# neverorfrog/vehicle-control

Hardware: AMD Instinct MI355X
Metric: MPC solves/sec (batched, N=20) (higher is better)
Workload: dtype f64; 1 GPU; C2 kinematic-bicycle LTV-MPC, B=1024 per GPU, N=20, fp64; batch_per_gpu=1024, global_batch=1024, horizon=20, parallelism=dp1 (independent shards)

## Files before the change

### vehicle-control_amd/csrc/kin_ltv.hip

```cpp
#include <hip/hip_runtime.h>

#include <cstdint>

#include "vc_kernels.hpp"
#include "vc_models.hpp"
#include "vcmpc.h"

#ifndef KIN_NU_TOL
#define KIN_NU_TOL 1e-10
#endif
#ifndef KIN_EARLY_F
#define KIN_EARLY_F 100.0
#endif
#ifndef KIN_EARLY_ROUNDS
#define KIN_EARLY_ROUNDS 2
#endif
#ifndef KIN_TAPIA_F
#define KIN_TAPIA_F 1.02
#endif
#ifndef KIN_DUAL_TOL
#define KIN_DUAL_TOL 1e-12
#endif
#ifndef KIN_AL_RHO
#define KIN_AL_RHO 1e1
#endif
#ifndef KIN_DOT_CH
#define KIN_DOT_CH 8
#endif
#ifndef KIN_UPDATE
#define KIN_UPDATE 1
#endif
#ifndef KIN_RSQ_HALLEY
#define KIN_RSQ_HALLEY 1
#endif
#ifndef KIN_STAT_CHECK
#define KIN_STAT_CHECK 0
#endif
#ifndef KIN_STEP_F
#define KIN_STEP_F 0.99
#endif
#ifndef KIN_SOLVE_CH
#define KIN_SOLVE_CH 8
#endif
#ifndef KIN_PANEL_CH
#define KIN_PANEL_CH 6
#endif

namespace vc {
namespace {

__device__ __forceinline__ double lane_bcast(double v, int src) {
  const int lo = __builtin_amdgcn_readlane(__double2loint(v), src);
  const int hi = __builtin_amdgcn_readlane(__double2hiint(v), src);
  return __hiloint2double(hi, lo);
}
__device__ int amdgcn_writelane(int v, int lane, int old) __asm("llvm.amdgcn.writelane.i32");
__device__ __forceinline__ double lane_put(double old, double v, int dst) {
  const int lo = amdgcn_writelane(__double2loint(v), dst, __double2loint(old));
  const int hi = amdgcn_writelane(__double2hiint(v), dst, __double2hiint(old));
  return __hiloint2double(hi, lo);
}
template <int K>
__device__ __forceinline__ double dpp_row_shr(double v, double ident) {
  const int lo = __builtin_amdgcn_update_dpp(__double2loint(ident), __double2loint(v), 0x110 + K, 0xf, 0xf, false);
  const int hi = __builtin_amdgcn_update_dpp(__double2hiint(ident), __double2hiint(v), 0x110 + K, 0xf, 0xf, false);
  return __hiloint2double(hi, lo);
}
template <typename Op>
__device__ __forceinline__ double wave_reduce(double v, double ident, Op op) {
  v = op(v, dpp_row_shr<1>(v, ident));
  v = op(v, dpp_row_shr<2>(v, ident));
  v = op(v, dpp_row_shr<4>(v, ident));
  v = op(v, dpp_row_shr<8>(v, ident));
  return op(op(lane_bcast(v, 15), lane_bcast(v, 31)), op(lane_bcast(v, 47), lane_bcast(v, 63)));
}
__device__ __forceinline__ double wave_sum(double v) {
  return wave_reduce(v, 0.0, [](double a, double b) { return a + b; });
}
__device__ __forceinline__ double wave_max(double v) {
  return wave_reduce(v, -__builtin_inf(), [](double a, double b) { return fmax(a, b); });
}
__device__ __forceinline__ double wave_min(double v) {
  return wave_reduce(v, __builtin_inf(), [](double a, double b) { return fmin(a, b); });
}
__device__ __forceinline__ void wave_sync() {
  asm volatile("" ::: "memory");
  __builtin_amdgcn_wave_barrier();
  asm volatile("" ::: "memory");
}
__device__ __forceinline__ void fence() { __builtin_amdgcn_sched_barrier(0); }
__device__ __forceinline__ int lane_opaque(int lane) {
  asm volatile("" : "+v"(lane));
  return lane;
}
__device__ __forceinline__ uint32_t lane_range_pick(uint32_t in, int other, int lo, int hi) {
  uint32_t r;
  asm("s_bfm_b64 vcc, %3, %4\n\t"
      "v_mov_b32_e32 %0, %2\n\tv_cndmask_b32_e32 %0, %0, %1, vcc"
      : "=&v"(r)
      : "v"(in), "i"(other), "i"(hi - lo), "i"(lo)
      : "vcc");
  return r;
}
__device__ __forceinline__ void no_hoist() { asm volatile("" ::: "memory"); }

using lds_cdouble = const __attribute__((address_space(3))) double;
__device__ __forceinline__ lds_cdouble* lds_opaque(const double* p) {
  uint32_t a = (uint32_t)(uintptr_t)(lds_cdouble*)p;
  asm volatile("" : "+v"(a));
  return (lds_cdouble*)(uintptr_t)a;
}

#ifdef VC_TIMING
#define VC_TSTAMP(var) \
  fence();              \
  const uint64_t var = __builtin_amdgcn_s_memtime(); \
  fence();
#define VC_TACC(slot, t0) \
  {                      \
    fence();             \
    tacc[slot] += __builtin_amdgcn_s_memtime() - (t0); \
    fence();             \
  }
#else
#define VC_TSTAMP(var)
#define VC_TACC(slot, t0)
#endif
enum { T_SWEEP = 0, T_SETUP, T_RESID, T_BUILD, T_CHOL, T_SOLVE, T_UPDATE, T_POLISH, T_OUT, T_S2, T_S3, T_S4, T_PAL, T_PPASS, T_NUPD, T_UCYC, T_NDROP, T_CFAIL, T_CRM, T_CADD, T_R0CHG, T_STEP, T_TOTAL, T_NSLOT };


template <int N>
struct Dims {
  static constexpr int n = 2 * N;
  static constexpr int NC = 2 * (N - 1);
  static constexpr int LD = n + 1;
  static_assert(n <= 64 && N >= 2, "one wavefront per problem needs 2 <= N <= 32");
};

template <int n>
__host__ __device__ constexpr int lc_base(int k) {
  static_assert(n % 2 == 0, "even n");
  return k * (n - 1) - k * (k - 1) / 2 + (k + 1) / 2;
}
template <int n>
__host__ __device__ constexpr int lc_start(int k) {
  return lc_base<n>(k) + k;
}

template <int N>
struct Smem {
  using D = Dims<N>;
  static constexpr int LC_DUMMY = lc_start<D::n>(D::n);
  static constexpr int LC_ZERO = LC_DUMMY + 1;
  double G[D::NC + 3][D::LD];
  double H[D::n + 1][D::LD];
  alignas(16) double Lc[LC_ZERO + 1];
  alignas(16) double zrow[48];
  double xb[N + 1][KIN_NX + 1];
  double jac[N + 1][9];
  double ub[D::n];
  double kap[N], ds[N];
  union {
    struct {
      double vz[64];
      double vc[64];
    };
    alignas(16) double tb2[128];
  };
  double dinv[64];
};

template <int N>
__host__ __device__ constexpr int crow_stage(int r) {
  return r < N - 1 ? r + 1 : r - (N - 1) + 1;
}

template <int LEN, int SA, int SB, int CH = KIN_DOT_CH>
__device__ __forceinline__ double lds_dot(lds_cdouble* a, lds_cdouble* b) {
  constexpr int NCH = (LEN + CH - 1) / CH;
  double ca[2][CH], cb[2][CH];
  auto fetch = [&](int c, int buf) {
#pragma unroll
    for (int q = 0; q < CH; ++q) {
      const int i = c * CH + q;
      ca[buf][q] = (i < LEN) ? a[i * SA] : 0.0;
      cb[buf][q] = (i < LEN) ? b[i * SB] : 0.0;
    }
  };
  double a0 = 0.0, a1 = 0.0;
  fetch(0, 0);
#pragma unroll
  for (int c = 0; c < NCH; ++c) {
    if (c + 1 < NCH) fetch(c + 1, (c + 1) & 1);
    fence();
#pragma unroll
    for (int q = 0; q < CH; q += 2) {
      a0 += ca[c & 1][q] * cb[c & 1][q];
      a1 += ca[c & 1][q + 1] * cb[c & 1][q + 1];
    }
  }
  fence();
  return a0 + a1;
}

template <int N>
__device__ double grow_dot(const Smem<N>& s, int lane) {
  constexpr int NC = Dims<N>::NC;
  const int r = lane < NC ? lane : 0;
  const double a = lds_dot<2 * (N - 1), 1, 1>(lds_opaque(&s.G[r][0]), lds_opaque(&s.vz[0]));
  return lane < NC ? a : 0.0;
}

template <int N>
__device__ double gt_dot(const Smem<N>& s, int lane) {
  constexpr int n = Dims<N>::n, NC = Dims<N>::NC, LD = Dims<N>::LD;
  const int j = lane < n ? lane : 0;
  const double a = lds_dot<NC, LD, 1>(lds_opaque(&s.G[0][j]), lds_opaque(&s.vc[0]));
  return lane < n ? a : 0.0;
}


template <int N>
__device__ double h_dot(const Smem<N>& s, int lane) {
  constexpr int n = Dims<N>::n;
  const int j = lane < n ? lane : 0;
  return lds_dot<n, 1, 1>(lds_opaque(&s.H[j][0]), lds_opaque(&s.vz[0]));
}

__device__ __forceinline__ void kin_sincos(double x, double& sn, double& cs) {
  const double n = __builtin_rint(x * 6.36619772367581382433e-01);
  const double y = fma(-n, 6.07710050650619224932e-11, fma(-n, 1.57079632673412561417e+00, x));
  const double z = y * y;
  const double rs = fma(z, fma(z, fma(z, fma(z, 1.58969099521155010221e-10, -2.50507602534068634195e-08),
                                      2.75573137070700676789e-06), -1.98412698298579493134e-04),
                        8.33333333332248946124e-03);
  const double sk = fma(z * y, fma(z, rs, -1.66666666666666324348e-01), y);
  const double rc = z * fma(z, fma(z, fma(z, fma(z, fma(z, -1.13596475577881948265e-11, 2.08757232129817482790e-09),
                                                  -2.75573143513906633035e-07), 2.48015872894767294178e-05),
                                   -1.38888888888741095749e-03), 4.16666666666666019037e-02);
  const double hz = 0.5 * z, w = 1.0 - hz;
  const double ck = w + (((1.0 - w) - hz) + z * rc);
  const int q = int(n) & 3;
  const double a = (q & 1) ? ck : sk, b = (q & 1) ? sk : ck;
  sn = (q & 2) ? -a : a;
  cs = ((q + 1) & 2) ? -b : b;
}

__device__ __forceinline__ double rsq_nr(double d) {
  double inv = __builtin_amdgcn_rsq(d);
#if KIN_RSQ_HALLEY
  const double e = fma(-d, inv * inv, 1.0);
  return fma(inv * e, fma(0.375, e, 0.5), inv);
#else
  inv = inv * (1.5 - 0.5 * d * inv * inv);
  inv = inv * (1.5 - 0.5 * d * inv * inv);
  return inv;
#endif
}

template <int N>
__device__ __forceinline__ void store_rows(const double (&Mr)[Dims<N>::n], Smem<N>& s, int lane) {
}

template <int N>
__device__ double chol_solve(const double (&Lr)[Dims<N>::n], const Smem<N>& s, double b, int lane) {
  constexpr int n = Dims<N>::n;
  constexpr int CH = KIN_SOLVE_CH;
  static_assert(n % CH == 0, "backward prefetch chunks");
  const int row = lane < n ? lane : 0;
  lds_cdouble* col = lds_opaque(&s.Lc[lc_base<n>(row)]);
  const double dj = s.dinv[row];
  double acc = b;
#pragma unroll
  for (int k = 0; k < n; ++k) acc -= Lr[k] * lane_bcast(acc * dj, k);
  acc *= dj;
  double x = 0.0;
  double lk[2][CH];
  lds_cdouble* zero = lds_opaque(&s.zrow[0]);
  auto fetch = [&](int c, int buf) {
    lds_cdouble* src = row < n - 1 - c * CH ? col : zero;
#pragma unroll
    for (int q = 0; q < CH; ++q) lk[buf][q] = src[n - 1 - c * CH - q];
  };
  fetch(0, 0);
#pragma unroll
  for (int c = 0; c < n / CH; ++c) {
    if (c + 1 < n / CH) fetch(c + 1, (c + 1) & 1);
    fence();
#pragma unroll
    for (int q = 0; q < CH; ++q) {
      const int k = n - 1 - c * CH - q;
      const double xk = lane_bcast(acc * dj, k);
      x = lane_put(x, xk, k);
      acc -= lk[c & 1][q] * xk;
    }
    fence();
  }
  return x;
}

enum { ROWS_G = 0, ROWS_E = 1 };
template <int N, int KIND>
__host__ __device__ constexpr int row_extent(int r) {
  if (KIND == ROWS_G) return r < Dims<N>::NC ? 2 * crow_stage<N>(r) : 0;
  return r < N ? 2 * (r + 1) : (r < N + 2 ? 2 * N : 0);
}
template <int N, int KIND>
__host__ __device__ constexpr int gram_rows() {
  return KIND == ROWS_G ? Dims<N>::NC : N + 2;
}
template <int N, int KIND>
__host__ __device__ constexpr bool kstep_hits(int ks, int I) {
  for (int q = 0; q < 4; ++q)
    if (row_extent<N, KIND>(4 * ks + q) > 16 * I) return true;
  return false;
}

using d4 = __attribute__((ext_vector_type(4))) double;
using d2 = __attribute__((ext_vector_type(2))) double;
template <int N>
struct Tiles {
  static constexpr int n = Dims<N>::n, NB = (n + 15) / 16, NT = NB * (NB + 1) / 2, BLD = 16 * NB + 2;
  static constexpr int count(bool full) { return full ? NB * NB : NT; }
};

template <int N, int KIND, bool FULL>
__device__ __forceinline__ void gram_mfma(d4 (&acc)[Tiles<N>::count(FULL)], const double* rows, const double* w,
                                          int lane) {
  constexpr int n = Dims<N>::n, LD = Dims<N>::LD, NB = Tiles<N>::NB;
  constexpr int KS = (gram_rows<N, KIND>() + 3) / 4;
  lane = lane_opaque(lane);
  const int lr = lane >> 4, lc = lane & 15;
  lds_cdouble* R = lds_opaque(rows);
  lds_cdouble* W = lds_opaque(w);
  double gk[KS][NB], wk[KS];
#pragma unroll
  for (int ks = 0; ks < KS; ++ks) {
    const int r = 4 * ks + lr;
    wk[ks] = W[r];
#pragma unroll
    for (int J = 0; J < NB; ++J) {
      const int c = 16 * J + lc;
      gk[ks][J] = R[r * LD + (c < n ? c : n)];
    }
  }
  fence();
#pragma unroll
  for (int ks = 0; ks < KS; ++ks) {
#pragma unroll
    for (int I = 0, t = 0; I < NB; ++I) {
      const double a = wk[ks] * gk[ks][I];
#pragma unroll
      for (int J = 0; J < (FULL ? NB : I + 1); ++J, ++t)
        if (kstep_hits<N, KIND>(ks, I > J ? I : J))
          acc[t] = __builtin_amdgcn_mfma_f64_16x16x4f64(a, gk[ks][J], acc[t], 0, 0, 0);
    }
  }
}

template <int N, bool FULL>
__device__ __forceinline__ void tiles_to_rows(double (&Mr)[Dims<N>::n], const d4 (&acc)[Tiles<N>::count(FULL)],
                                              Smem<N>& s, int lane) {
  constexpr int n = Dims<N>::n, NB = Tiles<N>::NB, BLD = Tiles<N>::BLD;
  static_assert(16 * BLD <= Smem<N>::LC_DUMMY, "transpose buffer must fit the factor storage");
  static_assert(16 * NB <= 48, "zero row length");
  lane = lane_opaque(lane);
  const int lr = lane >> 4, lc = lane & 15;
  double* buf = &s.Lc[0];
  const int myI = lane >> 4;
#pragma unroll
  for (int I = 0, t0 = 0; I < NB; ++I, t0 += FULL ? NB : I) {
    wave_sync();
#pragma unroll
    for (int J = 0; J < (FULL ? NB : I + 1); ++J) {
#pragma unroll
      for (int q = 0; q < 4; ++q) buf[(lr + 4 * q) * BLD + 16 * J + lc] = acc[t0 + J][q];
    }
    wave_sync();
    using lds_cd2 = const __attribute__((address_space(3))) d2;
    lds_cd2* brow = (lds_cd2*)lds_opaque(myI == I ? &buf[lc * BLD] : &s.zrow[0]);
#pragma unroll
    for (int i = 0; i < n; i += 2) {
      const int iend = FULL ? n : 16 * (I + 1);
      if (i < iend) {
        const d2 p = brow[i / 2];
        if (I == 0) { Mr[i] = p.x; Mr[i + 1] = p.y; }
        else { Mr[i] += p.x; Mr[i + 1] += p.y; }
      } else if (I == 0) {
        Mr[i] = 0.0;
        Mr[i + 1] = 0.0;
      }
    }
  }
  wave_sync();
}

template <int N>
__device__ __forceinline__ void build_normal_acc(d4 (&acc)[Tiles<N>::NT], Smem<N>& s, double wb, double hjj, int lane) {
  constexpr int n = Dims<N>::n, LD = Dims<N>::LD, NB = Tiles<N>::NB;
  static_assert(4 * ((Dims<N>::NC + 3) / 4) <= Dims<N>::NC + 2, "G zero rows cover the last k-step");
  lane = lane_opaque(lane);
  const int lr = lane >> 4, lc = lane & 15;
  const int jd = lane < n ? lane : n;
  s.H[jd][jd] = hjj + wb;
  wave_sync();
  {
    lds_cdouble* H = lds_opaque(&s.H[0][0]);
#pragma unroll
    for (int I = 0, t = 0; I < NB; ++I) {
#pragma unroll
      for (int J = 0; J <= I; ++J, ++t) {
        const int c = 16 * J + lc < n ? 16 * J + lc : n;
#pragma unroll
        for (int q = 0; q < 4; ++q) {
          const int r0 = 16 * I + 4 * q;
          acc[t][q] = r0 < n ? H[(r0 + lr) * LD + c] : 0.0;
        }
      }
    }
  }
  s.H[jd][jd] = hjj;
  gram_mfma<N, ROWS_G, false>(acc, &s.G[0][0], &s.vc[0], lane);
}

template <int N>
__device__ __forceinline__ void build_normal_mfma(double (&Mr)[Dims<N>::n], Smem<N>& s, double wb, double hjj,
                                                  int lane) {
  d4 acc[Tiles<N>::NT];
  build_normal_acc<N>(acc, s, wb, hjj, lane);
  tiles_to_rows<N, false>(Mr, acc, s, lane);
}

template <int N>
__device__ bool factor_blocked(double (&Mr)[Dims<N>::n], d4 (&acc)[Tiles<N>::NT], Smem<N>& s, int lane) {
  constexpr int n = Dims<N>::n, NB = Tiles<N>::NB;
  constexpr int DUMMY = Smem<N>::LC_DUMMY;
  static_assert(NB == 3 && n > 32 && n <= 40, "three panels, the last one at most 8 wide");
  static_assert(lc_start<n>(16) + 16 * 18 <= DUMMY, "panel 0/1 transpose buffer inside the factor storage");
  static_assert((lc_start<n>(16) & 1) == 0, "16-byte aligned transpose buffer");
  lane = lane_opaque(lane);
  const int lr = lane >> 4, lc = lane & 15, myI = lane >> 4;
  bool ok = true;
  double pa, pb, pc, pi1, pl21, pi2;
  using lds_double = __attribute__((address_space(3))) double;
  using lds_char = __attribute__((address_space(3))) char;
  const uint32_t lane8 = 8u * uint32_t(lane);
  auto col_store = [&](int k, double v) {
    const uint32_t off = lane_range_pick(lane8, 8 * (DUMMY - lc_base<n>(k)), k, n);
    *(lds_double*)((lds_char*)&s.Lc[lc_base<n>(k)] + off) = v;
  };
  auto part = [&](int p, int k) {
    if (p == 0) {
      pa = lane_bcast(Mr[k], k);
      pb = lane_bcast(Mr[k], k + 1);
      pc = lane_bcast(Mr[k + 1], k + 1);
      pi1 = rsq_nr(pa);
    } else if (p == 1) {
      pl21 = pb * pi1;
      const double d2 = fma(-pl21, pl21, pc);
      pi2 = rsq_nr(d2);
      ok = ok && (pa > 0.0) && (d2 > 0.0);
    } else {
      const double x = Mr[k] * pi1;
      const double y = fma(-x, pl21, Mr[k + 1]) * pi2;
      Mr[k] = x;
      Mr[k + 1] = y;
      col_store(k, x);
      col_store(k + 1, y);
      s.dinv[k] = pi1;
      s.dinv[k + 1] = pi2;
    }
  };
  using lds_cd2 = const __attribute__((address_space(3))) d2;
#pragma unroll
  for (int p = 0; p < NB; ++p) {
    const int c0 = 16 * p, c1 = (16 * p + 16 < n) ? 16 * p + 16 : n, W = c1 - c0;
    double* tb = p < 2 ? &s.Lc[lc_start<n>(16)] : &s.tb2[0];
    const int TS = p < 2 ? 18 : 10;
#pragma unroll
    for (int i = c0; i < c1; ++i) Mr[i] = 0.0;
#pragma unroll
    for (int I = p; I < NB; ++I) {
      const int t = I * (I + 1) / 2 + p;
      wave_sync();
#pragma unroll
      for (int q = 0; q < 4; ++q) {
        const int r = lr + 4 * q;
        if (4 * q < W)
          tb[(lc < W ? r * TS + lc : 8 * TS + lc)] = acc[t][q];
      }
      wave_sync();
      lds_cd2* src = (lds_cd2*)lds_opaque(myI == I && lc < W ? &tb[lc * TS] : &s.zrow[0]);
#pragma unroll
      for (int i = 0; i < W; i += 2) {
        const d2 v = src[i / 2];
        Mr[c0 + i] += v.x;
        Mr[c0 + i + 1] += v.y;
      }
    }
    wave_sync();
    part(0, c0);
    part(1, c0);
    part(2, c0);
#pragma unroll
    for (int k = c0; k + 2 < c1; k += 2) {
      wave_sync();
      fence();
      const double x = Mr[k], y = Mr[k + 1];
      const double* cA = &s.Lc[lc_base<n>(k)];
      const double* cB = &s.Lc[lc_base<n>(k + 1)];
      constexpr int CH = KIN_PANEL_CH;
      const int J0 = k + 4, NCH = (c1 - J0 + CH - 1) / CH;
      double u0[2][CH], u1[2][CH];
      auto load = [&](int ch, int buf) {
#pragma unroll
        for (int q = 0; q < CH; ++q) {
          const int j = J0 + ch * CH + q;
          u0[buf][q] = j < c1 ? cA[j] : 0.0;
          u1[buf][q] = j < c1 ? cB[j] : 0.0;
        }
      };
      if (NCH > 0) load(0, 0);
#pragma unroll
      for (int j = k + 2; j < k + 4; ++j)
        Mr[j] = fma(-y, lane_bcast(y, j), fma(-x, lane_bcast(x, j), Mr[j]));
      part(0, k + 2);
#pragma unroll
      for (int ch = 0; ch < NCH; ++ch) {
        if (ch + 1 < NCH) load(ch + 1, (ch + 1) & 1);
        fence();
#pragma unroll
        for (int q = 0; q < CH; ++q) {
          const int j = J0 + ch * CH + q;
          if (j < c1) Mr[j] = fma(-y, u1[ch & 1][q], fma(-x, u0[ch & 1][q], Mr[j]));
        }
        if (ch + 1 < 3) part(ch + 1, k + 2);
        fence();
      }
#pragma unroll
      for (int pp = NCH + 1; pp < 3; ++pp) {
        part(pp, k + 2);
        fence();
      }
    }
    wave_sync();
    if (p + 1 < NB) {
      lds_cdouble* Lc = lds_opaque(&s.Lc[0]);
      lds_cdouble* Z = lds_opaque(&s.zrow[0]);
#pragma unroll
      for (int ks = 0; ks < W / 4; ++ks) {
        const int kk = c0 + 4 * ks + lr;
        double op[NB];
#pragma unroll
        for (int I = p + 1; I < NB; ++I) {
          const int jj = 16 * I + lc;
          op[I] = jj < n ? Lc[lc_base<n>(kk) + jj] : Z[0];
        }
#pragma unroll
        for (int I = p + 1; I < NB; ++I) {
#pragma unroll
          for (int J = p + 1; J <= I; ++J) {
            const int t = I * (I + 1) / 2 + J;
            acc[t] = __builtin_amdgcn_mfma_f64_16x16x4f64(-op[I], op[J], acc[t], 0, 0, 0);
          }
        }
      }
    }
  }
#pragma unroll
  for (int k = 0; k < n; ++k) Mr[k] = lane_opaque(lane) > k ? Mr[k] : 0.0;
  store_rows<N>(Mr, s, lane);
  wave_sync();
  return ok;
}

__device__ __forceinline__ double wave_prefix(double v, int lane) {
  v += dpp_row_shr<1>(v, 0.0);
  v += dpp_row_shr<2>(v, 0.0);
  v += dpp_row_shr<4>(v, 0.0);
  v += dpp_row_shr<8>(v, 0.0);
  const double r0 = lane_bcast(v, 15), r1 = lane_bcast(v, 31), r2 = lane_bcast(v, 47);
  return v + (lane >= 16 ? r0 : 0.0) + (lane >= 32 ? r1 : 0.0) + (lane >= 48 ? r2 : 0.0);
}

template <int N>
__device__ bool factor_update(double (&Mr)[Dims<N>::n], Smem<N>& s, int upd, int j, bool fixed, double sqrho,
                              int lane) {
  constexpr int n = Dims<N>::n;
  constexpr int DUMMY = Smem<N>::LC_DUMMY, ZERO = Smem<N>::LC_ZERO;
  lane = lane_opaque(lane);
  const int row = lane < n ? lane : 0;
  auto below = [&](int k, int other) { return lane > k && lane < n ? lc_base<n>(k) + lane : other; };
  double z;
  if (upd == 1) {
    z = s.Lc[below(j, ZERO)];
    wave_sync();
    s.Lc[below(j, DUMMY)] = 0.0;
    s.Lc[lane < j ? lc_base<n>(lane) + j : DUMMY] = 0.0;
    s.Lc[lc_start<n>(j)] = 1.0;
    s.dinv[j] = 1.0;
  } else {
    z = (lane < n && !fixed) ? sqrho * s.G[j][lane < n ? lane : n] : 0.0;
  }
  wave_sync();
  {
    lds_cdouble* L = lds_opaque(&s.Lc[0]);
#pragma unroll
    for (int k = 0; k < n; ++k) Mr[k] = L[below(k, ZERO)];
  }
  const double dj = s.dinv[row];
  double acc = z;
#pragma unroll
  for (int k = 0; k < n; ++k) acc -= Mr[k] * lane_bcast(acc * dj, k);
  const double y = lane < n ? acc * dj : 0.0;
  const double t = 1.0 + wave_prefix(y * y, lane);
  const double sk = sqrt(t / (t - y * y)), ck = y / t;
  const bool ok = __ballot(!(sk > 0.5 && sk < 1e150)) == 0ull;
  wave_sync();
  if (lane < n) {
    s.Lc[lc_start<n>(row)] *= sk;
    s.dinv[row] = dj / sk;
  }
  s.tb2[2 * lane] = ck;
  s.tb2[2 * lane + 1] = sk;
  wave_sync();
  {
    using lds_cd2 = const __attribute__((address_space(3))) d2;
    lds_cd2* cs = (lds_cd2*)lds_opaque(&s.tb2[0]);
    double w = z;
#pragma unroll
    for (int k = 0; k < n - 1; ++k) {
      const double yk = lane_bcast(y, k);
      const d2 c = cs[k];
      w = lane_put(w, 0.0, k);
      const double l = Mr[k];
      w = fma(-yk, l, w);
      Mr[k] = fma(c.x, w, l) * c.y;
    }
  }
#pragma unroll
  for (int k = 0; k < n - 1; ++k) s.Lc[below(k, DUMMY)] = Mr[k];
  wave_sync();
  return ok;
}

struct Side {
  double lo, hi, slo, shi, llo, lhi;
  bool hasLo, hasHi;
};

}

template <int N>
__global__ __launch_bounds__(64) void kin_ltv_kernel(KinLtvArgs A) {
  using D = Dims<N>;
  constexpr int n = D::n, NC = D::NC;
  __shared__ Smem<N> s;
  const int lane = threadIdx.x;
  const int b = xcd_problem(blockIdx.x, A.B);
  if (b >= A.B) return;
  const vc_kin_mpc& W = A.w;
#ifdef VC_TIMING
  uint64_t tacc[T_NSLOT] = {};
#endif
  VC_TSTAMP(t_all0)

  if (lane < n) s.ub[lane] = A.ubar[(size_t)b * n + lane];
  if (lane < N) {
    s.kap[lane] = A.kappa[(size_t)b * N + lane];
    s.ds[lane] = A.ds[(size_t)b * N + lane];
  }
  if (lane < KIN_NX) s.xb[0][lane] = A.x0[(size_t)b * KIN_NX + lane];
  for (int i = lane; i < 2 * D::LD; i += 64) (&s.G[NC][0])[i] = 0.0;
  if (lane < 48) s.zrow[lane] = 0.0;
  if (lane == 0) s.Lc[Smem<N>::LC_ZERO] = 0.0;
  wave_sync();

  VC_TSTAMP(t_sweep0)
  constexpr int LD = Dims<N>::LD;
  double* E = &s.H[0][0];
  bool finite = true;
  {
    double x[KIN_NX];
#pragma unroll
    for (int i = 0; i < KIN_NX; ++i) x[i] = s.xb[0][i];
#pragma unroll 1
    for (int k = 0; k < N; ++k) {
      const double u2[2] = {s.ub[2 * k], s.ub[2 * k + 1]};
      const double h = s.ds[k];
      double f[KIN_NX];
      {
        double sn, cs;
        kin_sincos((lane & 1) ? x[1] : x[4], sn, cs);
        const double se = lane_bcast(sn, 0), ce = lane_bcast(cs, 0);
        const double sd = lane_bcast(sn, 1), cd = lane_bcast(cs, 1);
        const double kap = s.kap[k];
        const double rho = 1.0 - x[3] * kap;
        const int r4 = lane & 3;
        const double num = r4 == 0 ? se : (r4 == 1 ? sd : rho);
        const double den = r4 == 0 ? ce : (r4 == 1 ? cd * A.L : (r4 == 2 ? ce : x[0] * ce));
        const double quo = num * rcp_nr(den);
        const double te = lane_bcast(quo, 0), tdl = lane_bcast(quo, 1);
        const double rc = lane_bcast(quo, 2), q = lane_bcast(quo, 3);
        f[0] = q * u2[0];
        f[1] = q * u2[1];
        f[2] = 1.0;
        f[3] = rho * te;
        f[4] = tdl * rc - kap;
        f[5] = q;
      }
#pragma unroll
      for (int i = 0; i < KIN_NX; ++i) x[i] += h * f[i];
      if (lane == 0) {
#pragma unroll
        for (int i = 0; i < KIN_NX; ++i) s.xb[k + 1][i] = x[i];
      }
    }
#pragma unroll
    for (int i = 0; i < KIN_NX; ++i) finite = finite && isfinite(x[i]);
  }
  wave_sync();
  if (lane < N) {
    const double ey = s.xb[lane + 1][3];
    double cw, lin;
    if (lane + 1 < N) {
      const double hs = s.ds[lane + 1];
      const double td = W.w_dev * hs;
      double tb = W.w_b * hs;
      asm volatile("" : "+v"(tb));
      cw = td;
      lin = ey * td;
      if (ey < W.ey_min) { cw = __builtin_fma(W.w_dev, hs, tb); lin = __builtin_fma(ey - W.ey_min, tb, lin); }
      if (ey > W.ey_max) { cw = cw + tb; lin = __builtin_fma(ey - W.ey_max, tb, lin); }
    } else {
      cw = W.w_ey;
      lin = W.w_ey * ey;
    }
    s.vc[lane] = 2.0 * cw;
    s.vz[lane] = 2.0 * lin;
  }
  wave_sync();
  VC_TACC(T_SWEEP, t_sweep0)
  VC_TSTAMP(t_s20)
  {
    const int k = lane < N ? lane : 0;
    double xk[KIN_NX];
#pragma unroll
    for (int i = 0; i < KIN_NX; ++i) xk[i] = s.xb[k][i];
    const KinJac J = kin_spatial_jac(xk, s.kap[k], A.L);
    double* jr = s.jac[lane < N ? lane : N];
    jr[0] = J.q; jr[1] = J.qv; jr[2] = J.qey; jr[3] = J.qep;
    jr[4] = J.J33; jr[5] = J.J34; jr[6] = J.J41; jr[7] = J.J43; jr[8] = J.J44;
    if (A.obs.n > 0 && lane >= 1 && lane < N) {
      double p, q;
      obstacle_ey_model<double>(A.obs, xk[2], xk[3], W.w_obs * s.ds[k], p, q);
      s.vc[k - 1] += q;
      s.vz[k - 1] += p;
    }
  }
  wave_sync();
  VC_TACC(T_S2, t_s20)
  VC_TSTAMP(t_s30)
  double gj = 0.0;
  double cv = 0, cd = 0, cey = 0, cep = 0, ct = 0;
  {
    const int jcol = lane < n ? lane : n;
    double jn[9], hn, an, wn;
    auto fetch = [&](int k) {
#pragma unroll
      for (int q = 0; q < 9; ++q) jn[q] = s.jac[k][q];
      hn = s.ds[k]; an = s.ub[2 * k]; wn = s.ub[2 * k + 1];
    };
    fetch(0);
#pragma unroll 1
    for (int k = 0; k < N; ++k) {
      double J[9];
#pragma unroll
      for (int q = 0; q < 9; ++q) J[q] = jn[q];
      const double h = hn, a = an, w = wn;
      const double lin2 = s.vz[k];
      if (k + 1 < N) fetch(k + 1);
      const double dq = J[1] * cv + J[2] * cey + J[3] * cep;
      const double ncv = cv + h * a * dq + (lane == 2 * k ? h * J[0] : 0.0);
      const double ncd = cd + h * w * dq + (lane == 2 * k + 1 ? h * J[0] : 0.0);
      const double ncey = cey + h * (J[4] * cey + J[5] * cep);
      const double ncep = cep + h * (J[6] * cd + J[7] * cey + J[8] * cep);
      ct += h * dq;
      cv = ncv; cd = ncd; cey = ncey; cep = ncep;
      const bool has = k + 1 <= N - 1;
      s.G[has ? k : NC + 2][jcol] = cv;
      s.G[has ? (N - 1) + k : NC + 2][jcol] = cd;
      E[k * LD + jcol] = cey;
      gj += lin2 * cey;
    }
    E[N * LD + jcol] = cv;
    E[(N + 1) * LD + jcol] = cep;
  }
  wave_sync();
  VC_TACC(T_S3, t_s30)
  VC_TSTAMP(t_s40)
  double Hr[n];
  double hjj;
  {
    const double vN = s.xb[N][0];
    const double cwv = (vN >= W.v_max) ? W.w_v : 0.0;
    gj += 2.0 * cwv * (vN - W.v_max) * cv;
    gj += 2.0 * W.w_epsi * s.xb[N][4] * cep;
    gj += W.w_time * ct;
    if (lane < 4) s.vc[N + lane] = lane == 0 ? 2.0 * cwv : (lane == 1 ? 2.0 * W.w_epsi : 0.0);
    for (int i = lane; i < 2 * LD; i += 64) E[(N + 2) * LD + i] = 0.0;
    wave_sync();
    d4 acc[Tiles<N>::count(true)];
#pragma unroll
    for (int t = 0; t < Tiles<N>::count(true); ++t) acc[t] = d4{0.0, 0.0, 0.0, 0.0};
    gram_mfma<N, ROWS_E, true>(acc, E, &s.vc[0], lane);
    tiles_to_rows<N, true>(Hr, acc, s, lane);
  }
  const int kq = lane >> 1;
  double dself = 2.0 * A.qp.prox, dm2 = 0.0, dp2 = 0.0;
  if (lane < n) {
    if (lane & 1) {
      dself += 2.0 * W.w_w;
      gj += 2.0 * W.w_w * s.ub[lane];
    } else {
      if (kq >= 1) {
        dself += 2.0 * W.w_a; dm2 = -2.0 * W.w_a;
        gj += 2.0 * W.w_a * (s.ub[lane] - s.ub[lane - 2]);
      }
      if (kq <= N - 2) {
        dself += 2.0 * W.w_a; dp2 = -2.0 * W.w_a;
        gj -= 2.0 * W.w_a * (s.ub[lane + 2] - s.ub[lane]);
      }
    }
  }
  gj = (lane < n) ? gj : 0.0;
  {
    const int j = lane < n ? lane : n;
#pragma unroll
    for (int i = 0; i < n; ++i) s.H[j][i] = Hr[i];
    s.H[j][n] = 0.0;
    s.H[j][j] += dself;
    s.H[j][j >= 2 ? j - 2 : j] += dm2;
    s.H[j][j + 2 < n ? j + 2 : j] += dp2;
    hjj = lane < n ? s.H[j][j] : 0.0;
  }
  wave_sync();
  if (A.mode == 1) {
    if (lane < n) {
#pragma unroll
      for (int i = 0; i < n; ++i) A.H_out[((size_t)b * n + lane) * n + i] = s.H[lane][i];
      A.g_out[(size_t)b * n + lane] = gj;
    }
    return;
  }

  VC_TACC(T_S4, t_s40)
  VC_TSTAMP(t_setup0)
  Side bx, cs;
  {
    const bool isw = lane & 1;
    const double u = (lane < n) ? s.ub[lane] : 0.0;
    bx.lo = (isw ? W.w_min : W.a_min) - u;
    bx.hi = (isw ? W.w_max : W.a_max) - u;
    const double tr = isw ? A.qp.trust_w : A.qp.trust_a;
    if (tr > 0.0) {
      bx.lo = fmax(bx.lo, -tr);
      bx.hi = fmin(bx.hi, tr);
    }
    bx.hasLo = bx.hasHi = (lane < n);
    const int st = crow_stage<N>(lane < NC ? lane : 0);
    if (lane < N - 1) {
      cs.lo = W.v_min - s.xb[st][0];
      cs.hi = 0.0;
      cs.hasLo = true; cs.hasHi = false;
    } else if (lane < NC) {
      cs.lo = W.delta_min - s.xb[st][1];
      cs.hi = W.delta_max - s.xb[st][1];
      cs.hasLo = cs.hasHi = true;
    } else {
      cs.lo = cs.hi = 0.0;
      cs.hasLo = cs.hasHi = false;
    }
  }
  const double mtot = double(4 * N + 3 * (N - 1));
  double scale, hdiag_max;
  {
    double m = fabs(gj);
    if (bx.hasLo) m = fmax(m, fabs(bx.lo));
    if (bx.hasHi) m = fmax(m, fabs(bx.hi));
    if (cs.hasLo) m = fmax(m, fabs(cs.lo));
    if (cs.hasHi) m = fmax(m, fabs(cs.hi));
    scale = 1.0 + wave_max(m);
    hdiag_max = fmax(wave_max(hjj), 1.0);
  }
  double z = 0.0;
  bx.slo = bx.hasLo ? fmax(-bx.lo, 1.0) : 1.0;
  bx.shi = bx.hasHi ? fmax(bx.hi, 1.0) : 1.0;
  bx.llo = bx.hasLo ? 1.0 : 0.0;
  bx.lhi = bx.hasHi ? 1.0 : 0.0;
  cs.slo = cs.hasLo ? fmax(-cs.lo, 1.0) : 1.0;
  cs.shi = cs.hasHi ? fmax(cs.hi, 1.0) : 1.0;
  cs.llo = cs.hasLo ? 1.0 : 0.0;
  cs.lhi = cs.hasHi ? 1.0 : 0.0;

  VC_TACC(T_SETUP, t_setup0)
  const int max_iter = A.qp.max_iter;
  const double tol = A.qp.tol * scale;
  int it = 0;
  bool converged = false, chol_fail = false, near = false;
  double last_res = 0.0, last_mu = 0.0;
  double Mr[n];
  double rd = 0.0, rlo_b = 0.0, rhi_b = 0.0, rlo_c = 0.0, rhi_c = 0.0;
  auto true_residuals = [&]() {
    wave_sync();
    s.vz[lane] = (lane < n) ? z : 0.0;
    s.vc[lane] = (lane < NC) ? (cs.lhi - cs.llo) : 0.0;
    wave_sync();
    const double yc = grow_dot<N>(s, lane);
    rd = (lane < n) ? (h_dot<N>(s, lane) + gj + (bx.lhi - bx.llo) + gt_dot<N>(s, lane)) : 0.0;
    rlo_b = bx.hasLo ? (z - bx.lo - bx.slo) : 0.0;
    rhi_b = bx.hasHi ? (bx.hi - z - bx.shi) : 0.0;
    rlo_c = cs.hasLo ? (yc - cs.lo - cs.slo) : 0.0;
    rhi_c = cs.hasHi ? (cs.hi - yc - cs.shi) : 0.0;
  };
  auto max_residual = [&]() {
    return wave_max(fmax(fmax(fabs(rd), fmax(fabs(rlo_b), fabs(rhi_b))), fmax(fabs(rlo_c), fabs(rhi_c))));
  };
  int tapb = 0;
  const double tol_early = KIN_EARLY_F > 0.0 ? fmax(tol, KIN_EARLY_F * tol) : tol;
  int e_set = 0;
#ifdef VC_TIMING
  uint64_t e_fmask = 0;
  bool e_row = false, e_have = false;
#endif
  double tol_cur = tol_early;
  bool polished = false, pchol_fail = false;
  int rounds = 0;
#pragma unroll 1
  for (;;) {
  if (finite) {
#pragma unroll 1
    for (;;) {
      no_hoist();
      VC_TSTAMP(t_res0)
      if (it == 0) true_residuals();
      const double mu = wave_sum(bx.slo * bx.llo + bx.shi * bx.lhi + cs.slo * cs.llo + cs.shi * cs.lhi) / mtot;
      double res = max_residual();
      if (it > 0 && res <= tol_cur && mu <= tol_cur) {
        true_residuals();
        res = max_residual();
      }
      converged = res <= tol_cur && mu <= tol_cur;
      last_res = res;
      last_mu = mu;
      if (converged || it >= max_iter || !isfinite(res) || !isfinite(mu)) break;
      ++it;
      const double wlo_b = bx.hasLo ? bx.llo / bx.slo : 0.0;
      const double whi_b = bx.hasHi ? bx.lhi / bx.shi : 0.0;
      const double wlo_c = cs.hasLo ? cs.llo / cs.slo : 0.0;
      const double whi_c = cs.hasHi ? cs.lhi / cs.shi : 0.0;
      wave_sync();
      s.vc[lane] = (lane < NC) ? wlo_c + whi_c : 0.0;
      wave_sync();
      VC_TACC(T_RESID, t_res0)
      VC_TSTAMP(t_build0)
      d4 nacc[Tiles<N>::NT];
      build_normal_acc<N>(nacc, s, wlo_b + whi_b, hjj, lane);
      VC_TACC(T_BUILD, t_build0)
      VC_TSTAMP(t_chol0)
      const bool chol_ok = factor_blocked<N>(Mr, nacc, s, lane);
      VC_TACC(T_CHOL, t_chol0)
      if (!chol_ok) {
        chol_fail = true;
        near = res <= 1e-6 * scale && mu <= tol;
        break;
      }
#ifdef VC_TIMING
      const uint64_t t_sol_before = tacc[T_SOLVE];
#endif
      VC_TSTAMP(t_step0)
      const double islo_b = bx.hasLo ? rcp_nr(bx.slo) : 0.0, ishi_b = bx.hasHi ? rcp_nr(bx.shi) : 0.0;
      const double islo_c = cs.hasLo ? rcp_nr(cs.slo) : 0.0, ishi_c = cs.hasHi ? rcp_nr(cs.shi) : 0.0;
      const double illo_b = bx.hasLo ? rcp_nr(bx.llo) : 0.0, ilhi_b = bx.hasHi ? rcp_nr(bx.lhi) : 0.0;
      const double illo_c = cs.hasLo ? rcp_nr(cs.llo) : 0.0, ilhi_c = cs.hasHi ? rcp_nr(cs.lhi) : 0.0;
      double sm = 0.0, pp1 = 0.0, pp2 = 0.0, pp3 = 0.0, pp4 = 0.0;
#pragma unroll 1
      for (int pass = 0; pass < 2; ++pass) {
        no_hoist();
        const double rclo_b = bx.slo * bx.llo + pp1 - sm, rchi_b = bx.shi * bx.lhi + pp2 - sm;
        const double rclo_c = cs.slo * cs.llo + pp3 - sm, rchi_c = cs.shi * cs.lhi + pp4 - sm;
        const double eb = (bx.hasHi ? (-rchi_b * ishi_b - whi_b * rhi_b) : 0.0) +
                          (bx.hasLo ? (rclo_b * islo_b + wlo_b * rlo_b) : 0.0);
        const double ec = (cs.hasHi ? (-rchi_c * ishi_c - whi_c * rhi_c) : 0.0) +
                          (cs.hasLo ? (rclo_c * islo_c + wlo_c * rlo_c) : 0.0);
        wave_sync();
        s.vc[lane] = (lane < NC) ? ec : 0.0;
        wave_sync();
        const double rhs = (lane < n) ? (-rd - eb - gt_dot<N>(s, lane)) : 0.0;
        VC_TSTAMP(t_sol0)
        const double dz = chol_solve<N>(Mr, s, rhs, lane);
        VC_TACC(T_SOLVE, t_sol0)
        wave_sync();
        s.vz[lane] = (lane < n) ? dz : 0.0;
        wave_sync();
        const double dyc = grow_dot<N>(s, lane);
        const double d1 = bx.hasLo ? dz + rlo_b : 0.0;
        const double d2 = bx.hasLo ? (-rclo_b * islo_b - wlo_b * (dz + rlo_b)) : 0.0;
        const double d3 = bx.hasHi ? rhi_b - dz : 0.0;
        const double d4 = bx.hasHi ? (-rchi_b * ishi_b - whi_b * (rhi_b - dz)) : 0.0;
        const double e1 = cs.hasLo ? dyc + rlo_c : 0.0;
        const double e2 = cs.hasLo ? (-rclo_c * islo_c - wlo_c * (dyc + rlo_c)) : 0.0;
        const double e3 = cs.hasHi ? rhi_c - dyc : 0.0;
        const double e4 = cs.hasHi ? (-rchi_c * ishi_c - whi_c * (rhi_c - dyc)) : 0.0;
        const double tmax = wave_max(fmax(fmax(fmax(-d1 * islo_b, -d2 * illo_b), fmax(-d3 * ishi_b, -d4 * ilhi_b)),
                                          fmax(fmax(-e1 * islo_c, -e2 * illo_c), fmax(-e3 * ishi_c, -e4 * ilhi_c))));
        const double amax = 1.0 / fmax(1.0, tmax);
        if (pass == 0) {
          const double mua = wave_sum((bx.slo + amax * d1) * (bx.llo + amax * d2) +
                                      (bx.shi + amax * d3) * (bx.lhi + amax * d4) +
                                      (cs.slo + amax * e1) * (cs.llo + amax * e2) +
                                      (cs.shi + amax * e3) * (cs.lhi + amax * e4)) / mtot;
          const double sr = mua / mu;
          sm = sr * sr * sr * mu;
          pp1 = d1 * d2; pp2 = d3 * d4; pp3 = e1 * e2; pp4 = e3 * e4;
        } else {
          const double al = KIN_STEP_F * amax;
          {
            auto tap = [&](double dl, double il, double dsv, double is) -> int {
              const double lr = fma(al * dl, il, 1.0), sr = fma(al * dsv, is, 1.0);
              return lr > KIN_TAPIA_F * sr ? 1 : (sr > KIN_TAPIA_F * lr ? 2 : 0);
            };
            tapb = tap(d2, illo_b, d1, islo_b) | (tap(d4, ilhi_b, d3, ishi_b) << 2) |
                   (tap(e2, illo_c, e1, islo_c) << 4) | (tap(e4, ilhi_c, e3, ishi_c) << 6);
          }
          z = (lane < n) ? z + al * dz : z;
          bx.slo += al * d1; bx.llo += al * d2; bx.shi += al * d3; bx.lhi += al * d4;
          cs.slo += al * e1; cs.llo += al * e2; cs.shi += al * e3; cs.lhi += al * e4;
          const double om = 1.0 - al;
          rd *= om; rlo_b *= om; rhi_b *= om; rlo_c *= om; rhi_c *= om;
        }
      }
      VC_TACC(T_STEP, t_step0)
#ifdef VC_TIMING
      tacc[T_STEP] -= tacc[T_SOLVE] - t_sol_before;
#endif
    }
  }

  VC_TSTAMP(t_pol0)
  if ((converged || near) && A.qp.polish > 0) {
    constexpr double AL_RHO = KIN_AL_RHO;
    constexpr int AL_MAX = 16;
    const double ptol = 1e-9 * scale, dtol = KIN_DUAL_TOL * scale;
    auto guess = [&](bool has, double l, double sv, int t) { return has && (t == 1 || (t == 0 && l > sv)); };
    bool alo_b = guess(bx.hasLo, bx.llo, bx.slo, tapb & 3);
    bool ahi_b = guess(bx.hasHi, bx.lhi, bx.shi, (tapb >> 2) & 3);
    bool alo_c = guess(cs.hasLo, cs.llo, cs.slo, (tapb >> 4) & 3);
    bool ahi_c = guess(cs.hasHi, cs.lhi, cs.shi, (tapb >> 6) & 3);
    auto pack = [&]() { return int(alo_b) | (int(ahi_b) << 1) | (int(alo_c) << 2) | (int(ahi_c) << 3); };
    if (tol_cur <= tol && __ballot(e_set != 0 && pack() != (e_set & 15)) == 0ull && __ballot(e_set != 0) != 0ull) {
      const int t = e_set >> 4;
      alo_b = t & 1; ahi_b = (t >> 1) & 1; alo_c = (t >> 2) & 1; ahi_c = (t >> 3) & 1;
    }
    const int max_rounds = tol_cur > tol ? min(A.qp.polish, KIN_EARLY_ROUNDS) : A.qp.polish;
    double rho_k = 0.0;
    int upd = 0, upd_j = 0;
#pragma unroll 1
    for (int round = 0; round < max_rounds; ++round) {
      no_hoist();
      const int set0 = pack();
#ifdef VC_TIMING
      if (round == 0 && tol_cur <= tol && e_have) {
        const bool fx = (lane < n) && (alo_b || ahi_b);
        const uint64_t fm = __ballot(fx);
        const bool ract = (lane < NC) && (alo_c || ahi_c);
        tacc[T_CFAIL] = 1;
        tacc[T_CRM] = __builtin_popcountll(e_fmask & ~fm) + __builtin_popcountll(__ballot(e_row && !ract));
        tacc[T_CADD] = __builtin_popcountll(fm & ~e_fmask) + __builtin_popcountll(__ballot(ract && !e_row));
      }
#endif
      ++rounds;
      const bool fixed = (lane < n) && (alo_b || ahi_b);
      const double zfix = fixed ? (alo_b ? bx.lo : bx.hi) : 0.0;
      const uint64_t fmask = __ballot(fixed);
      const bool act = (lane < NC) && (alo_c || ahi_c);
      wave_sync();
      s.vz[lane] = (lane < n) ? zfix : 0.0;
      wave_sync();
      const double gfix = grow_dot<N>(s, lane);
      double gn2 = 0.0;
      {
        const int r = lane < NC ? lane : 0;
#pragma unroll 2
        for (int i = 0; i < 2 * (N - 1); ++i) {
          const double gi = ((fmask >> i) & 1ull) ? 0.0 : s.G[r][i];
          gn2 += gi * gi;
        }
      }
      const double rho_new = (act && gn2 > 1e-28) ? AL_RHO * hdiag_max / gn2 : 0.0;
      const double rho_c = (KIN_UPDATE && rho_k > 0.0 && rho_new > 0.0) ? rho_k : rho_new;
      const double bnd_c = act ? ((alo_c ? cs.lo : cs.hi) - gfix) : 0.0;
      const double base = (lane < n) ? -(gj + h_dot<N>(s, lane)) : 0.0;
      wave_sync();
      s.vc[lane] = rho_c;
      wave_sync();
      VC_TSTAMP(t_pf0)
      bool updated = false;
      if (KIN_UPDATE && upd != 0) {
        const bool same = __ballot(lane < NC && rho_c != rho_k && !(upd == 2 && lane == upd_j)) == 0ull;
        VC_TSTAMP(t_u0)
        if (same) updated = factor_update<N>(Mr, s, upd, upd_j, fixed, sqrt(lane_bcast(rho_c, upd_j)), lane);
#ifdef VC_TIMING
        if (updated) tacc[T_NUPD] += 1;
#endif
        VC_TACC(T_UCYC, t_u0)
      }
      rho_k = rho_c;
      if (!updated) {
        d4 pacc[Tiles<N>::NT];
        build_normal_acc<N>(pacc, s, 0.0, hjj, lane);
        const int pl = lane_opaque(lane), plr = pl >> 4, plc = pl & 15;
#pragma unroll
        for (int I = 0, t = 0; I < Tiles<N>::NB; ++I) {
#pragma unroll
          for (int J = 0; J <= I; ++J, ++t) {
            const int c = 16 * J + plc;
            const bool fc = (fmask >> c) & 1ull;
#pragma unroll
            for (int q = 0; q < 4; ++q) {
              const int r = 16 * I + plr + 4 * q;
              const bool fr = (fmask >> r) & 1ull;
              pacc[t][q] = (fr || fc) ? (r == c ? 1.0 : 0.0) : pacc[t][q];
            }
          }
        }
        if (!factor_blocked<N>(Mr, pacc, s, lane)) {
          pchol_fail = true;
          break;
        }
      }
      VC_TACC(T_UPDATE, t_pf0)
      VC_TSTAMP(t_pal0)
      double nu_c = (act && rho_c > 0.0) ? ((ahi_c ? cs.lhi : 0.0) - (alo_c ? cs.llo : 0.0)) : 0.0;

      const bool al_act = act && rho_c > 0.0;
      const double bnd_al = alo_c ? cs.lo : cs.hi;
      double zp = 0.0, emax = 0.0;
      {
        wave_sync();
        s.vc[lane] = (lane < NC) ? (nu_c - rho_c * bnd_c) : 0.0;
        wave_sync();
        const double rhs = (lane < n) ? (fixed ? zfix : (base - gt_dot<N>(s, lane))) : 0.0;
        zp = chol_solve<N>(Mr, s, rhs, lane);
        wave_sync();
        s.vz[lane] = (lane < n) ? zp : 0.0;
        wave_sync();
        const double yr = grow_dot<N>(s, lane);
        double rr = al_act ? (yr - bnd_al) : 0.0;
        const double ie = 1.0 / (1e-14 * scale), inu = KIN_NU_TOL > 0.0 ? 1.0 / (KIN_NU_TOL * scale) : 0.0;
        auto crit = [&](double r) { return wave_max(fmax(fabs(r) * ie, fabs(rho_c * r) * inu)); };
#ifdef VC_TIMING
        tacc[T_PPASS] += 1;
#endif
        if (crit(rr) > 1.0) {
          double pd = rho_c * rr;
          double rz = wave_sum(rr * pd);
#pragma unroll 1
          for (int it = 1; it < AL_MAX; ++it) {
            no_hoist();
            wave_sync();
            s.vc[lane] = (lane < NC) ? pd : 0.0;
            wave_sync();
            const double gtp = gt_dot<N>(s, lane);
            const double zq = chol_solve<N>(Mr, s, (lane < n && !fixed) ? gtp : 0.0, lane);
            wave_sync();
            s.vz[lane] = (lane < n) ? zq : 0.0;
            wave_sync();
            const double gq = grow_dot<N>(s, lane);
            const double q = al_act ? gq : 0.0;
            const double pq = wave_sum(pd * q);
#ifdef VC_TIMING
            tacc[T_PPASS] += 1;
#endif
            if (!(pq > 0.0)) break;
            const double al = rz / pq;
            nu_c = fma(al, pd, nu_c);
            zp = fma(-al, zq, zp);
            rr = fma(-al, q, rr);
            if (crit(rr) <= 1.0) break;
            const double zt = rho_c * rr;
            const double rzn = wave_sum(rr * zt);
            pd = fma(rzn / rz, pd, zt);
            rz = rzn;
          }
        }
      }
      VC_TACC(T_PAL, t_pal0)
      wave_sync();
      s.vz[lane] = (lane < n) ? zp : 0.0;
      s.vc[lane] = (lane < NC) ? nu_c : 0.0;
      wave_sync();
      const double grad = (lane < n) ? (h_dot<N>(s, lane) + gj + gt_dot<N>(s, lane)) : 0.0;
      const double ypc = grow_dot<N>(s, lane);
#if KIN_STAT_CHECK
      emax = wave_max(fmax(al_act ? fabs(ypc - bnd_al) : 0.0, (lane < n && !fixed) ? fabs(grad) : 0.0));
#else
      emax = wave_max(al_act ? fabs(ypc - bnd_al) : 0.0);
#endif
      const double dv_b = (lane < n) ? (ahi_b ? grad : (alo_b ? -grad : -1.0)) : -1.0;
      const double dv_c = (lane < NC) ? (ahi_c ? -nu_c : (alo_c ? nu_c : -1.0)) : -1.0;
      const double pv_b = (lane < n && !fixed) ? fmax(bx.lo - zp, zp - bx.hi) : -1.0;
      const double pv_c = (lane < NC && !(act && rho_c > 0.0))
                              ? fmax(cs.hasLo ? cs.lo - ypc : -1.0, cs.hasHi ? ypc - cs.hi : -1.0)
                              : -1.0;
      const double dmax = wave_max(fmax(dv_b, dv_c));
      const double pmax = wave_max(fmax(pv_b, pv_c));
      if (dmax <= dtol && pmax <= ptol) {
        if (emax <= ptol) {
          z = (lane < n) ? zp : z;
          polished = true;
        }
        break;
      }
      const bool dual = dmax > dtol;
      const double worst = dual ? dmax : pmax;
      const double vb = dual ? dv_b : pv_b, vcr = dual ? dv_c : pv_c;
      const uint64_t who = __ballot(fmax(vb, vcr) == worst);
      const int sel = __builtin_ffsll((long long)who) - 1;
      const bool sel_box = (__ballot(vb >= vcr) >> sel) & 1ull;
      upd = dual ? 0 : (sel_box ? 1 : 2);
      upd_j = sel;
#ifdef VC_TIMING
      if (dual) tacc[T_NDROP] += 1;
#endif
      if (lane == sel) {
        if (vb >= vcr) {
          if (dual) { alo_b = false; ahi_b = false; }
          else if (zp < bx.lo) alo_b = true;
          else ahi_b = true;
        } else {
          if (dual) { alo_c = false; ahi_c = false; }
          else if (ypc < cs.lo) alo_c = true;
          else ahi_c = true;
        }
      }
#ifdef VC_TIMING
      int r0code = 0;
      if (tol_cur > tol && round == 0) {
        int tside = 0;
        if (vb >= vcr) tside = (dual ? (ahi_b ? (tapb >> 2) : tapb) : (zp < bx.lo ? tapb : (tapb >> 2))) & 3;
        else tside = (dual ? (ahi_c ? (tapb >> 6) : (tapb >> 4)) : (ypc < cs.lo ? (tapb >> 4) : (tapb >> 6))) & 3;
        const int code = 1 + (dual ? 2 : (vb >= vcr ? 0 : 1)) + 3 * tside;
        r0code = __builtin_amdgcn_readlane(code, sel);
#ifdef VC_TIMING
        tacc[T_R0CHG] = (uint64_t)r0code;
#endif
      }
#endif
      if (tol_cur > tol) e_set = 256 | set0 | (pack() << 4);
#ifdef VC_TIMING
      if (tol_cur > tol) {
        e_fmask = fmask;
        e_row = rho_k > 0.0;
        e_have = true;
      }
#endif
    }
  }

  VC_TACC(T_POLISH, t_pol0)
  if (polished || !converged || chol_fail || tol_cur <= tol) break;
  tol_cur = tol;
  converged = false;
  pchol_fail = false;
  }
  VC_TSTAMP(t_out0)
  int32_t st;
  if (!finite) st = VC_NONFINITE;
  else if (polished || converged) st = VC_SOLVED;
  else st = VC_MAX_ITER;
  if (!finite) z = 0.0;
  wave_sync();
  if (lane < n) {
    s.vz[lane] = z;
    A.u_out[(size_t)b * n + lane] = s.ub[lane] + z;
  }
  wave_sync();
  if (lane < 2) A.u0[(size_t)b * 2 + lane] = s.ub[lane] + s.vz[lane];
  if (lane == 0) {
    A.status[b] = st;
    A.iters[b] = it;
    if (A.diag) {
#ifdef VC_TIMING
      constexpr size_t DS = 4 + T_NSLOT;
#else
      constexpr size_t DS = 4;
#endif
      A.diag[(size_t)b * DS + 0] = last_res / scale;
      A.diag[(size_t)b * DS + 1] = last_mu / scale;
      A.diag[(size_t)b * DS + 2] = double((chol_fail ? 1 : 0) | (converged ? 2 : 0) | (polished ? 4 : 0) |
                                          (pchol_fail ? 8 : 0));
      A.diag[(size_t)b * DS + 3] = double(rounds);
    }
  }
  {
    const double y = grow_dot<N>(s, lane);
    const int slot = lane < N - 1 ? 64 + lane + 1
                                  : (lane < NC ? n + (lane - (N - 1)) + 1 : (lane == NC ? 64 : (lane == NC + 1 ? n : 127)));
    wave_sync();
    s.tb2[slot] = y;
    wave_sync();
    double ey = 0.0, ep = 0.0, eyk = 0.0, epk = 0.0;
#pragma unroll 4
    for (int k = 0; k < N; ++k) {
      const double h = s.ds[k], dd = s.vz[n + k];
      eyk = lane_put(eyk, ey, k);
      epk = lane_put(epk, ep, k);
      const double ney = ey + h * (s.jac[k][4] * ey + s.jac[k][5] * ep);
      const double nep = ep + h * (s.jac[k][6] * dd + s.jac[k][7] * ey + s.jac[k][8] * ep);
      ey = ney; ep = nep;
    }
    eyk = lane_put(eyk, ey, N);
    epk = lane_put(epk, ep, N);
    const double eyn = __shfl_down(eyk, 1), epn = __shfl_down(epk, 1);
    const int k = lane < N ? lane : 0;
    const double q = s.jac[k][0], qv = s.jac[k][1], qey = s.jac[k][2], qep = s.jac[k][3];
    const double h = s.ds[k], a = s.ub[2 * k], w = s.ub[2 * k + 1];
    const double da = s.vz[2 * k], dw = s.vz[2 * k + 1];
    const double dv = s.vc[k], dd = s.vz[n + k];
    const double dq = qv * dv + qey * eyk + qep * epk;
    const double dt = wave_prefix(lane < N ? h * dq : 0.0, lane);
    wave_sync();
    if (lane < N) {
      double* xr = s.xb[k + 1];
      xr[0] += dv + h * (a * dq + q * da);
      xr[1] += dd + h * (w * dq + q * dw);
      xr[3] += eyn;
      xr[4] += epn;
      xr[5] += dt;
    }
    wave_sync();
    double* xo = A.x_out + (size_t)b * (N + 1) * KIN_NX;
    for (int i = lane; i < (N + 1) * KIN_NX; i += 64) xo[i] = s.xb[i / KIN_NX][i % KIN_NX];
  }
  VC_TACC(T_OUT, t_out0)
  VC_TACC(T_TOTAL, t_all0)
#ifdef VC_TIMING
  if (A.diag && lane < T_NSLOT) {
    double v = 0.0;
#pragma unroll
    for (int i = 0; i < T_NSLOT; ++i) v = (i == lane) ? double(tacc[i]) : v;
    A.diag[(size_t)b * (4 + T_NSLOT) + 4 + lane] = v;
  }
#endif
}

size_t kin_ltv_smem_bytes(int N) {
  switch (N) {
    case 20: return sizeof(Smem<20>);
    default: return 0;
  }
}

hipError_t launch_kin_ltv(const KinLtvArgs& a, int N, hipStream_t stream) {
  if (a.B <= 0) return hipSuccess;
  switch (N) {
    case 20:
      hipLaunchKernelGGL(kin_ltv_kernel<20>, dim3(a.B), dim3(64), 0, stream, a);
      return hipGetLastError();
    default:
      return hipErrorInvalidValue;
  }
}

}
```

Baseline: 5.388 million solves/s.

## Transpose all panel blocks in one sync round and use explicit FMAs

The panel Cholesky staging now writes every block row of a panel into separate LDS buffers between a single pair of wave barriers, then has each lane read only its own block. The old code ran one barrier-separated transpose round per block row and accumulated into zeroed registers. A small extra LDS buffer is added and a static assert on per-problem LDS size is introduced. The residual and predictor-corrector arithmetic is rewritten with explicit fused multiply-adds, and fences are placed around a dot product, which may change rounding and instruction scheduling slightly.

Result: faster. 5.443 million solves/s (median of 6 runs) (+1.0%).

```diff
diff --git a/vehicle-control_amd/csrc/kin_ltv.hip b/vehicle-control_amd/csrc/kin_ltv.hip
--- a/vehicle-control_amd/csrc/kin_ltv.hip
+++ b/vehicle-control_amd/csrc/kin_ltv.hip
@@ -44,6 +44,10 @@
 #endif
 #ifndef KIN_PANEL_CH
 #define KIN_PANEL_CH 6
+#endif
+
+#ifndef KIN_XPOSE_ONCE
+#define KIN_XPOSE_ONCE 1
 #endif
 
 namespace vc {
@@ -168,7 +172,11 @@
     alignas(16) double tb2[128];
   };
   double dinv[64];
+#if KIN_XPOSE_ONCE
+  alignas(16) double tb3[8 * 18];
+#endif
 };
+static_assert(sizeof(Smem<20>) <= 40960, "LDS of one problem: four must fit a CU's 160 KB");
 
 template <int N>
 __host__ __device__ constexpr int crow_stage(int r) {
@@ -477,6 +485,36 @@
     const int c0 = 16 * p, c1 = (16 * p + 16 < n) ? 16 * p + 16 : n, W = c1 - c0;
     double* tb = p < 2 ? &s.Lc[lc_start<n>(16)] : &s.tb2[0];
     const int TS = p < 2 ? 18 : 10;
+#if KIN_XPOSE_ONCE
+    static_assert(2 * 16 * 18 + 8 * 18 <= DUMMY, "panel 0's three buffers inside the factor storage");
+    {
+      auto tbuf = [&](int I) -> double* {
+        return p == 0 ? &s.Lc[16 * 18 * I] : (p == 1 ? (I == 1 ? tb : &s.tb3[0]) : tb);
+      };
+      wave_sync();
+#pragma unroll
+      for (int I = p; I < NB; ++I) {
+        const int t = I * (I + 1) / 2 + p;
+        double* tbI = tbuf(I);
+#pragma unroll
+        for (int q = 0; q < 4; ++q) {
+          const int r = lr + 4 * q;
+          if (16 * I + 4 * q < n)
+            tbI[(lc < W ? r * TS + lc : 8 * TS + lc)] = acc[t][q];
+        }
+      }
+      wave_sync();
+      const double* own = p == 0 ? &s.Lc[16 * 18 * myI + lc * TS]
+                                 : (p == 1 ? (myI == 1 ? &tb[lc * TS] : &s.tb3[lc * TS]) : &tb[lc * TS]);
+      lds_cd2* src = (lds_cd2*)lds_opaque(myI >= p && lane < n ? own : &s.zrow[0]);
+#pragma unroll
+      for (int i = 0; i < W; i += 2) {
+        const d2 v = src[i / 2];
+        Mr[c0 + i] = 0.0 + v.x;
+        Mr[c0 + i + 1] = 0.0 + v.y;
+      }
+    }
+#else
 #pragma unroll
     for (int i = c0; i < c1; ++i) Mr[i] = 0.0;
 #pragma unroll
@@ -498,6 +536,7 @@
         Mr[c0 + i + 1] += v.y;
       }
     }
+#endif
     wave_sync();
     part(0, c0);
     part(1, c0);
@@ -917,7 +956,10 @@
     s.vc[lane] = (lane < NC) ? (cs.lhi - cs.llo) : 0.0;
     wave_sync();
     const double yc = grow_dot<N>(s, lane);
-    rd = (lane < n) ? (h_dot<N>(s, lane) + gj + (bx.lhi - bx.llo) + gt_dot<N>(s, lane)) : 0.0;
+    fence();
+    const double hz = h_dot<N>(s, lane);
+    fence();
+    rd = (lane < n) ? (hz + gj + (bx.lhi - bx.llo) + gt_dot<N>(s, lane)) : 0.0;
     rlo_b = bx.hasLo ? (z - bx.lo - bx.slo) : 0.0;
     rhi_b = bx.hasHi ? (bx.hi - z - bx.shi) : 0.0;
     rlo_c = cs.hasLo ? (yc - cs.lo - cs.slo) : 0.0;
@@ -944,7 +986,9 @@
       no_hoist();
       VC_TSTAMP(t_res0)
       if (it == 0) true_residuals();
-      const double mu = wave_sum(bx.slo * bx.llo + bx.shi * bx.lhi + cs.slo * cs.llo + cs.shi * cs.lhi) / mtot;
+      const double mu = wave_sum(__builtin_fma(cs.shi, cs.lhi,
+                                               __builtin_fma(cs.slo, cs.llo,
+                                                             __builtin_fma(bx.shi, bx.lhi, bx.slo * bx.llo)))) / mtot;
       double res = max_residual();
       if (it > 0 && res <= tol_cur && mu <= tol_cur) {
         true_residuals();
@@ -987,12 +1031,14 @@
 #pragma unroll 1
       for (int pass = 0; pass < 2; ++pass) {
         no_hoist();
-        const double rclo_b = bx.slo * bx.llo + pp1 - sm, rchi_b = bx.shi * bx.lhi + pp2 - sm;
-        const double rclo_c = cs.slo * cs.llo + pp3 - sm, rchi_c = cs.shi * cs.lhi + pp4 - sm;
-        const double eb = (bx.hasHi ? (-rchi_b * ishi_b - whi_b * rhi_b) : 0.0) +
-                          (bx.hasLo ? (rclo_b * islo_b + wlo_b * rlo_b) : 0.0);
-        const double ec = (cs.hasHi ? (-rchi_c * ishi_c - whi_c * rhi_c) : 0.0) +
-                          (cs.hasLo ? (rclo_c * islo_c + wlo_c * rlo_c) : 0.0);
+        const double rclo_b = __builtin_fma(bx.slo, bx.llo, pp1) - sm, rchi_b = __builtin_fma(bx.shi, bx.lhi, pp2) - sm;
+        const double rclo_c = __builtin_fma(cs.slo, cs.llo, pp3) - sm, rchi_c = __builtin_fma(cs.shi, cs.lhi, pp4) - sm;
+        const double thi_b = ishi_b * -rchi_b, thi_c = ishi_c * -rchi_c;
+        const double tlo_b = islo_b * rclo_b, tlo_c = islo_c * rclo_c;
+        const double eb = (bx.hasHi ? __builtin_fma(-whi_b, rhi_b, thi_b) : 0.0) +
+                          (bx.hasLo ? __builtin_fma(wlo_b, rlo_b, tlo_b) : 0.0);
+        const double ec = (cs.hasHi ? __builtin_fma(-whi_c, rhi_c, thi_c) : 0.0) +
+                          (cs.hasLo ? __builtin_fma(wlo_c, rlo_c, tlo_c) : 0.0);
         wave_sync();
         s.vc[lane] = (lane < NC) ? ec : 0.0;
         wave_sync();
@@ -1005,13 +1051,13 @@
         wave_sync();
         const double dyc = grow_dot<N>(s, lane);
         const double d1 = bx.hasLo ? dz + rlo_b : 0.0;
-        const double d2 = bx.hasLo ? (-rclo_b * islo_b - wlo_b * (dz + rlo_b)) : 0.0;
+        const double d2 = bx.hasLo ? __builtin_fma(islo_b, -rclo_b, -(wlo_b * (dz + rlo_b))) : 0.0;
         const double d3 = bx.hasHi ? rhi_b - dz : 0.0;
-        const double d4 = bx.hasHi ? (-rchi_b * ishi_b - whi_b * (rhi_b - dz)) : 0.0;
+        const double d4 = bx.hasHi ? __builtin_fma(-whi_b, rhi_b - dz, thi_b) : 0.0;
         const double e1 = cs.hasLo ? dyc + rlo_c : 0.0;
-        const double e2 = cs.hasLo ? (-rclo_c * islo_c - wlo_c * (dyc + rlo_c)) : 0.0;
+        const double e2 = cs.hasLo ? __builtin_fma(islo_c, -rclo_c, -(wlo_c * (dyc + rlo_c))) : 0.0;
         const double e3 = cs.hasHi ? rhi_c - dyc : 0.0;
-        const double e4 = cs.hasHi ? (-rchi_c * ishi_c - whi_c * (rhi_c - dyc)) : 0.0;
+        const double e4 = cs.hasHi ? __builtin_fma(-whi_c, rhi_c - dyc, thi_c) : 0.0;
         const double tmax = wave_max(fmax(fmax(fmax(-d1 * islo_b, -d2 * illo_b), fmax(-d3 * ishi_b, -d4 * ilhi_b)),
                                           fmax(fmax(-e1 * islo_c, -e2 * illo_c), fmax(-e3 * ishi_c, -e4 * ilhi_c))));
         const double amax = 1.0 / fmax(1.0, tmax);
```
